# cc-ai/MUNIT

Measured on AMD Instinct MI355X. Metric: images/sec (gen_update+dis_update) @256x256 bs=8, higher is better.
Workload: dtype f32; 1 GPU; config_256.yaml AdaINGen_double+MsImageDis dis_update+gen_update, 256x256, per-GPU batch 8, fp32; global_batch=8, parallelism=dp1, gen_state=1

## Files before the change

munit_amd/csrc/conv_igemm.hip:

```cpp
#include "common.h"
#include "wino.h"
#include <cstdlib>

namespace {

struct IgemmParams {
  const float* x;
  const float* w;
  const float* bias;
  void* y;
  int B, H, W, Cin;
  int Hu, Wu, ups;
  int Ho, Wo, Cout;
  int KH, KW, stride, pad, reflect;
  int Ktot;
  long long w_row;
  long long y_sb;
  long long y_sh;
  int y_sw;
  int M;
  int act;
  float slope;
  int ps;
  long long w_phase;
// ... 952 lines not shown

int check_desc(const munit_conv_desc* d) {
  MUNIT_CHECK_ARG(d != nullptr, "conv: null descriptor");
  MUNIT_CHECK_ARG(d->B > 0 && d->H > 0 && d->W > 0 && d->Cin > 0 && d->Cout > 0, "conv: bad dims");
  MUNIT_CHECK_ARG(d->KH > 0 && d->KW > 0 && d->stride > 0 && d->pad >= 0, "conv: bad kernel geometry");
  MUNIT_CHECK_ARG(d->upsample == 0 || d->upsample == 1, "conv: upsample must be 0 or 1");
  MUNIT_CHECK_ARG(d->compute >= MUNIT_COMPUTE_F32 && d->compute <= MUNIT_COMPUTE_F32X3, "conv: bad compute mode %d", d->compute);
  MUNIT_CHECK_ARG(d->pad_mode == MUNIT_PAD_ZERO || d->pad_mode == MUNIT_PAD_REFLECT, "conv: bad pad mode");
  MUNIT_CHECK_ARG((d->in_dtype == MUNIT_DTYPE_F32 || d->in_dtype == MUNIT_DTYPE_BF16) &&
                  (d->out_dtype == MUNIT_DTYPE_F32 || d->out_dtype == MUNIT_DTYPE_BF16), "conv: bad tensor dtype");
  MUNIT_CHECK_ARG(d->in_dtype == MUNIT_DTYPE_F32 || d->Cin % 64 == 0, "conv: a bf16 input needs Cin %% 64 == 0 (got %d)", d->Cin);
  MUNIT_CHECK_ARG(d->out_dtype == MUNIT_DTYPE_F32 || d->Cout % 64 == 0, "conv: a bf16 output needs Cout %% 64 == 0 (got %d)", d->Cout);
  const int Hu = d->H << d->upsample, Wu = d->W << d->upsample;
  if (d->pad_mode == MUNIT_PAD_REFLECT)
    MUNIT_CHECK_ARG(d->pad < Hu && d->pad < Wu, "conv: reflect pad %d needs input > pad (got %dx%d)", d->pad, Hu, Wu);
  MUNIT_CHECK_ARG(Hu + 2 * d->pad >= d->KH && Wu + 2 * d->pad >= d->KW, "conv: kernel larger than padded input");
  MUNIT_CHECK_ARG((long long)d->B * Hu * Wu < (1ll << 31) / 4, "conv: too many pixels for 32-bit tile indices");
  MUNIT_CHECK_ARG((long long)d->B * (Hu + 2 * d->pad) * (Wu + 2 * d->pad) * std::max(d->Cin, d->Cout) < (1ll << 31),
                  "conv: tensor too large for the 32-bit element offsets of the tile loader");
  return MUNIT_OK;
}

}

extern "C" int munit_conv2d_out_hw(const munit_conv_desc* d, int* Ho, int* Wo) {
  int rc = check_desc(d);
  if (rc) return rc;
  *Ho = ((d->H << d->upsample) + 2 * d->pad - d->KH) / d->stride + 1;
  *Wo = ((d->W << d->upsample) + 2 * d->pad - d->KW) / d->stride + 1;
  return MUNIT_OK;
}

namespace {
bool subpixel_ok(const munit_conv_desc* d) {
  return d->upsample == 1 && d->KH == 5 && d->KW == 5 && d->pad == 2 && d->stride == 1 &&
         d->pad_mode == MUNIT_PAD_REFLECT && d->Cin % 32 == 0 && d->H >= 3 && d->W >= 3 &&
         !MUNIT_ENV_FLAG("MUNIT_DEBUG_NO_SUBPIXEL");
}
}

namespace {
__global__ void pad3to4_image_kernel(const float* __restrict__ x, f32x4* __restrict__ x4, long long npix) {
  for (long long i = (long long)blockIdx.x * blockDim.x + threadIdx.x; i < npix; i += (long long)gridDim.x * blockDim.x)
    x4[i] = f32x4{x[3 * i], x[3 * i + 1], x[3 * i + 2], 0.f};
}
__global__ void pad3to4_weight_kernel(const float* __restrict__ w, float* __restrict__ w4, int N, int taps, int kpad) {
  const long long total = (long long)N * kpad;
  for (long long i = (long long)blockIdx.x * blockDim.x + threadIdx.x; i < total; i += (long long)gridDim.x * blockDim.x) {
    const int n = (int)(i / kpad), k = (int)(i - (long long)n * kpad);
    const int tap = k >> 2, c = k & 3;
    w4[i] = (tap < taps && c < 3) ? w[((long long)n * taps + tap) * 3 + c] : 0.f;
  }
}
struct Cin4Plan {
  int kpad;
  size_t x4_bytes, w4_bytes;
};
Cin4Plan plan_cin4(long long npix, int N, int taps) {
  Cin4Plan c;
  c.kpad = (taps * 4 + BK - 1) / BK * BK;
  c.x4_bytes = align_up((size_t)npix * 4 * sizeof(float), 256);
  c.w4_bytes = align_up((size_t)N * c.kpad * sizeof(float), 256);
  return c;
}
int build_cin4(const Cin4Plan& c, const float* x3, long long npix, const float* w3, int N, int taps, void* ws, hipStream_t st) {
  f32x4* x4 = reinterpret_cast<f32x4*>(ws);
  float* w4 = reinterpret_cast<float*>(reinterpret_cast<char*>(ws) + c.x4_bytes);
  hipLaunchKernelGGL(pad3to4_image_kernel, dim3((unsigned)std::min<long long>((npix + 255) / 256, 8192)), dim3(256), 0, st, x3, x4, npix);
  MUNIT_CHECK_LAUNCH("pad3to4_image");
  hipLaunchKernelGGL(pad3to4_weight_kernel, dim3((unsigned)cdiv((long long)N * c.kpad, 256)), dim3(256), 0, st, w3, w4, N, taps, c.kpad);
  MUNIT_CHECK_LAUNCH("pad3to4_weight");
  return MUNIT_OK;
}
bool cin4_fwd_ok(const munit_conv_desc* d) {
  return d->Cin == 3 && d->in_dtype == MUNIT_DTYPE_F32 && d->upsample == 0 && d->KH * d->KW <= 64 && d->Cout % 4 == 0 &&
         NWAVES == 8 && !MUNIT_ENV_FLAG("MUNIT_DEBUG_NO_CIN4");
}

bool wino_geometry_ok(const munit_conv_desc* d) {
  return d->compute == MUNIT_COMPUTE_F32 && d->in_dtype == MUNIT_DTYPE_F32 && d->out_dtype == MUNIT_DTYPE_F32 &&
         d->KH == 3 && d->KW == 3 && d->stride == 1 && d->pad == 1 && d->upsample == 0 && d->act != MUNIT_ACT_TANH;
}
bool wino_fwd_ok(const munit_conv_desc* d) { return wino_geometry_ok(d) && munit_wino_ok(d->B, d->H, d->W, d->Cin, d->Cout); }
long long wino_s2_min_blocks() {
  static const long long v = getenv("MUNIT_WINO_S2_MIN_BLOCKS") ? atoll(getenv("MUNIT_WINO_S2_MIN_BLOCKS")) : 192;
  return v;
}
long long wino_s2_dgrad_min_blocks() {
  static const long long v = getenv("MUNIT_WINO_S2_MIN_BLOCKS") ? atoll(getenv("MUNIT_WINO_S2_MIN_BLOCKS")) : 100;
  return v;
}
bool wino_s2_fwd_ok(const munit_conv_desc* d) {
  return d->compute == MUNIT_COMPUTE_F32 && d->in_dtype == MUNIT_DTYPE_F32 && d->out_dtype == MUNIT_DTYPE_F32 && d->KH == 4 &&
         d->KW == 4 && d->stride == 2 && d->pad == 1 && d->upsample == 0 && d->act != MUNIT_ACT_TANH && d->H >= 4 && d->W >= 4 &&
         munit_wino_ok(d->B, d->H, d->W, d->Cin, d->Cout) && !MUNIT_ENV_FLAG("MUNIT_DEBUG_NO_WINOGRAD_S2") &&
         (long long)cdiv((long long)d->B * cdiv(d->H / 2, 3) * cdiv(d->W / 2, 3), 64) * (d->Cout / 64) >= wino_s2_min_blocks();
}
bool wino_s2_dgrad_ok(const munit_conv_desc* d) {
  if (!(d->compute == MUNIT_COMPUTE_F32 && d->in_dtype == MUNIT_DTYPE_F32 && d->out_dtype == MUNIT_DTYPE_F32 && d->KH == 4 &&
        d->KW == 4 && d->stride == 2 && d->pad == 1 && d->upsample == 0 && d->H >= 4 && d->W >= 4 && d->H % 2 == 0 && d->W % 2 == 0 &&
        d->Cout % 8 == 0 && d->Cin % 64 == 0 && !MUNIT_ENV_FLAG("MUNIT_DEBUG_NO_WINOGRAD_S2") && !MUNIT_ENV_FLAG("MUNIT_DEBUG_NO_WINOGRAD")))
    return false;
  const int Hd = d->H / 2, Wd = d->W / 2;
  if (d->pad_mode == MUNIT_PAD_REFLECT && (Hd % 3 == 0 || Wd % 3 == 0)) return false;
  if ((long long)d->B * d->H * d->W * std::max(d->Cin, d->Cout) >= (1ll << 29)) return false;
  return (long long)cdiv((long long)d->B * cdiv(Hd + 1, 3) * cdiv(Wd + 1, 3), 64) * (d->Cin / 64) * 4 >= wino_s2_dgrad_min_blocks();
}
bool subpixel_wino_ok(const munit_conv_desc* d) {
  return subpixel_ok(d) && d->compute == MUNIT_COMPUTE_F32 && d->in_dtype == MUNIT_DTYPE_F32 && d->out_dtype == MUNIT_DTYPE_F32 &&
         d->act != MUNIT_ACT_TANH && munit_wino_ok(d->B, d->H, d->W, d->Cin, d->Cout);
}

munit_prep_item fwd_prep_item(const munit_conv_desc* d, const float* w, float* wp) {
  munit_prep_item it{w, wp, d->Cout, d->KH, d->KW, d->Cin, MUNIT_PREP_NONE, 1, 0};
  const bool small = munit_small_fwd_supported(d) && !MUNIT_ENV_FLAG("MUNIT_DEBUG_NO_SMALL_FWD");
  if (small) return it;
  it.bf16 = d->in_dtype == MUNIT_DTYPE_BF16;
  if (subpixel_ok(d)) it.kind = subpixel_wino_ok(d) ? MUNIT_PREP_SUBPIXEL_WINOGRAD : MUNIT_PREP_SUBPIXEL;
  else if (wino_fwd_ok(d)) it.kind = MUNIT_PREP_WINOGRAD;
  else if (wino_s2_fwd_ok(d)) it.kind = MUNIT_PREP_WINOGRAD_S2;
  else if (it.bf16) it.kind = MUNIT_PREP_CAST;
  return it;
}
size_t prep_bytes(const munit_prep_item& it) {
  return it.kind == MUNIT_PREP_NONE ? 0 : align_up((size_t)prep_elems(it) * (it.bf16 ? 2 : 4), 256);
}
}

extern "C" size_t munit_conv2d_fwd_workspace_bytes(const munit_conv_desc* d) {
  int Ho, Wo;
  if (munit_conv2d_out_hw(d, &Ho, &Wo)) return 0;
  const size_t img = prep_bytes(fwd_prep_item(d, nullptr, nullptr));
  if (munit_small_fwd_supported(d) && !MUNIT_ENV_FLAG("MUNIT_DEBUG_NO_SMALL_FWD")) return munit_small_fwd_workspace(d);
  if (munit_small_fwd_supported(d) || d->in_dtype == MUNIT_DTYPE_BF16 || wino_fwd_ok(d) || wino_s2_fwd_ok(d)) return img;
  if (cin4_fwd_ok(d)) {
    const Cin4Plan c = plan_cin4((long long)d->B * d->H * d->W, d->Cout, d->KH * d->KW);
    return c.x4_bytes + c.w4_bytes;
  }
  if (subpixel_ok(d))
    return img + std::max(splitk_bytes(d->B * (4 * Wo + 4 * (Ho - 4)), d->Cout, d->KH * d->KW * d->Cin, 1),
                          splitk_bytes(d->B * (2 * Wo + 2 * (Ho - 2)), d->Cout, d->KH * d->KW * d->Cin, 1));
  return img + splitk_bytes(d->B * Ho * Wo, d->Cout, d->KH * d->KW * d->Cin, 1);
}

extern "C" int munit_conv2d_fwd(const munit_conv_desc* d, const void* x, const float* w,
                                const float* bias, void* y, void* ws, size_t ws_bytes,
                                munit_stream_t stream) {
  return munit_conv2d_fwd_prepared(d, x, w, nullptr, bias, y, ws, ws_bytes, stream);
}

extern "C" int munit_conv2d_fwd_prepared(const munit_conv_desc* d, const void* x, const float* w, const void* wp,
                                         const float* bias, void* y, void* ws, size_t ws_bytes,
                                         munit_stream_t stream) {
  int Ho, Wo;
  int rc = munit_conv2d_out_hw(d, &Ho, &Wo);
  if (rc) return rc;
  MUNIT_CHECK_ARG(x && w && y, "conv2d_fwd: null pointer");
  hipStream_t st = (hipStream_t)stream;
  if (munit_small_fwd_supported(d) && !MUNIT_ENV_FLAG("MUNIT_DEBUG_NO_SMALL_FWD")) {
    MUNIT_CHECK_ARG(d->out_dtype == MUNIT_DTYPE_F32, "conv2d_fwd: the 3-channel image head writes fp32");
    const size_t sneed = munit_small_fwd_workspace(d);
    if (sneed != 0 && (ws == nullptr || ws_bytes < sneed)) {
      munit_set_error("conv2d_fwd: workspace %zu < %zu", ws_bytes, sneed);
      return MUNIT_ERR_WORKSPACE;
    }
    return munit_small_fwd(d, Ho, Wo, x, w, bias, reinterpret_cast<float*>(y), ws, st);
  }
  const size_t need = munit_conv2d_fwd_workspace_bytes(d);
  if (need != 0 && (ws == nullptr || ws_bytes < need)) {
    munit_set_error("conv2d_fwd: workspace %zu < %zu", ws_bytes, need);
    return MUNIT_ERR_WORKSPACE;
  }
  munit_prep_item it = fwd_prep_item(d, w, reinterpret_cast<float*>(ws));
  const size_t img_bytes = prep_bytes(it);
  const float* wimg = w;
  if (it.kind != MUNIT_PREP_NONE) {
    wimg = reinterpret_cast<const float*>(wp);
    if (wimg == nullptr) {
      rc = launch_prep_one(it, st);
      if (rc) return rc;
      wimg = it.wp;
    }
  }
  if (it.kind == MUNIT_PREP_WINOGRAD_S2) {
    WinoParams q{};
    q.x = reinterpret_cast<const float*>(x); q.u = wimg; q.bias = bias; q.y = reinterpret_cast<float*>(y);
    q.y_sw = d->Cout; q.y_sh = (long long)Wo * d->Cout; q.y_sb = (long long)Ho * Wo * d->Cout;
    q.B = d->B; q.H = d->H; q.W = d->W; q.K = 4 * d->Cin; q.N = d->Cout; q.xc = d->Cin; q.cpp = d->Cin / 8;
    q.s2 = 1; q.Ho = Ho; q.Wo = Wo;
    q.x_bytes = (unsigned)((size_t)d->B * d->H * d->W * d->Cin * 4);
    q.mode = d->pad_mode == MUNIT_PAD_REFLECT ? 0 : 1;
    q.th = cdiv(Ho, 3); q.tw = cdiv(Wo, 3); q.bth = cdiv(q.th, 8); q.btw = cdiv(q.tw, 8); q.NB = d->Cout / 64;
    q.act = d->act; q.slope = d->slope;
    return munit_wino_launch(q, st);
  }
  if (it.kind == MUNIT_PREP_WINOGRAD) {
    WinoParams q{};
    q.x = reinterpret_cast<const float*>(x); q.u = wimg; q.bias = bias; q.y = reinterpret_cast<float*>(y);
    q.y_sw = d->Cout; q.y_sh = (long long)d->W * d->Cout; q.y_sb = (long long)d->H * d->W * d->Cout;
    q.B = d->B; q.H = d->H; q.W = d->W; q.K = d->Cin; q.N = d->Cout; q.xc = d->Cin; q.cpp = d->Cin / 8;
    q.x_bytes = (unsigned)((size_t)d->B * d->H * d->W * d->Cin * 4);
    q.mode = d->pad_mode == MUNIT_PAD_REFLECT ? 0 : 1;
    q.th = d->H / 2; q.tw = d->W / 2; q.bth = cdiv(q.th, 8); q.btw = cdiv(q.tw, 8); q.NB = d->Cout / 64;
    q.act = d->act; q.slope = d->slope;
    return munit_wino_launch(q, st);
  }
  void* slabs = ws ? reinterpret_cast<char*>(ws) + img_bytes : nullptr;
  const size_t slab_bytes = ws ? ws_bytes - img_bytes : 0;
  IgemmParams p{};
  p.x = reinterpret_cast<const float*>(x); p.w = wimg; p.bias = bias; p.y = y;
  p.B = d->B; p.H = d->H; p.W = d->W; p.Cin = d->Cin;
  p.ups = d->upsample; p.Hu = d->H << p.ups; p.Wu = d->W << p.ups;
  p.Ho = Ho; p.Wo = Wo; p.Cout = d->Cout;
  p.KH = d->KH; p.KW = d->KW; p.stride = d->stride; p.pad = d->pad;
  p.reflect = d->pad_mode == MUNIT_PAD_REFLECT;
  p.Ktot = d->KH * d->KW * d->Cin;
  p.w_row = p.Ktot;
  p.y_sw = d->Cout;
  p.y_sh = (long long)Wo * d->Cout;
  p.y_sb = (long long)Ho * Wo * d->Cout;
  p.M = d->B * Ho * Wo;
  p.act = d->act; p.slope = d->slope;
  p.ct = d->compute;
  p.ps = 1;
  p.bf16s = d->in_dtype == MUNIT_DTYPE_BF16;
  p.out_bf16 = d->out_dtype == MUNIT_DTYPE_BF16;
  if (cin4_fwd_ok(d)) {
    const long long npix = (long long)d->B * d->H * d->W;
    const Cin4Plan c = plan_cin4(npix, d->Cout, d->KH * d->KW);
    rc = build_cin4(c, reinterpret_cast<const float*>(x), npix, w, d->Cout, d->KH * d->KW, ws, st);
    if (rc) return rc;
    p.x = reinterpret_cast<const float*>(ws);
    p.w = reinterpret_cast<const float*>(reinterpret_cast<const char*>(ws) + c.x4_bytes);
    p.Ktot = c.kpad; p.w_row = c.kpad; p.cin4 = 1;
    return launch_igemm<0>(p, 1, st);
  }
  if (it.kind == MUNIT_PREP_SUBPIXEL || it.kind == MUNIT_PREP_SUBPIXEL_WINOGRAD) {
    IgemmParams q = p;
    int ring = 2;
    q.ups = 0; q.Hu = d->H; q.Wu = d->W;
    q.Ho = d->H; q.Wo = d->W;
    q.KH = 3; q.KW = 3; q.pad = 1; q.reflect = 0;
    q.Ktot = 9 * d->Cin; q.w_row = q.Ktot;
    q.y_sw = 2 * d->Cout;
    q.y_sh = (long long)2 * Wo * d->Cout;
    q.M = d->B * d->H * d->W;
    q.ps = 2;
    q.w_phase = (long long)d->Cout * q.Ktot;
    q.y_phase_row = (long long)Wo * d->Cout;
    q.y_phase_col = d->Cout;
    if (it.kind == MUNIT_PREP_SUBPIXEL_WINOGRAD) {
      WinoParams wq{};
      wq.x = reinterpret_cast<const float*>(x); wq.u = wimg; wq.bias = bias; wq.y = reinterpret_cast<float*>(y);
      wq.y_sw = q.y_sw; wq.y_sh = q.y_sh; wq.y_sb = p.y_sb;
      wq.u_phase = wino_image_elems(d->Cin, d->Cout); wq.y_prow = q.y_phase_row; wq.y_pcol = q.y_phase_col; wq.phases = 4;
      wq.B = d->B; wq.H = d->H; wq.W = d->W; wq.K = d->Cin; wq.N = d->Cout; wq.xc = d->Cin; wq.cpp = d->Cin / 8;
      wq.x_bytes = (unsigned)((size_t)d->B * d->H * d->W * d->Cin * 4);
      wq.mode = 1;
      wq.edge = 1;
      ring = 1;
      wq.th = d->H / 2; wq.tw = d->W / 2; wq.bth = cdiv(wq.th, 8); wq.btw = cdiv(wq.tw, 8); wq.NB = d->Cout / 64;
      wq.act = d->act; wq.slope = d->slope;
      rc = munit_wino_launch(wq, st);
    } else {
      rc = launch_igemm<0>(q, 4, st);
    }
    if (rc) return rc;
    p.frame = ring;
    p.M = d->B * (2 * ring * Wo + 2 * ring * (Ho - 2 * ring));
    p.w = it.bf16 ? reinterpret_cast<const float*>(reinterpret_cast<const bf16_t*>(wimg) + (size_t)4 * 9 * d->Cout * d->Cin) : w;
    return launch_igemm<0>(p, 1, st, slabs, slab_bytes);
  }
  return launch_igemm<0>(p, 1, st, slabs, slab_bytes);
}

namespace {
__global__ void box2x2_kernel(const f32x4* __restrict__ dy, f32x4* __restrict__ s, int B, int H, int W, int C4) {
// ... 506 lines not shown
```

munit_amd/csrc/conv_wino.hip:

```cpp
#include "wino.h"
#include <algorithm>
#include <type_traits>

namespace {

constexpr int WT = 64;
constexpr int WNB = 64;
constexpr int WK = 8;
constexpr int VBUF = 16 * WT * WK;
constexpr int UBUF = 16 * WNB * WK;
constexpr int MLD = 36;
constexpr int WINO_SMEM = 16 * WT * MLD;
static_assert(WINO_SMEM >= 2 * VBUF, "operand buffers must fit");

typedef float f32x2 __attribute__((ext_vector_type(2)));

#ifdef WINO_STAMP
__device__ long long g_wino_stamps[8 * 8 * 4];
#define WSTAMP(i) do { const long long t_ = __builtin_amdgcn_s_memtime(); st_acc[i] += t_ - st_last; st_last = t_; } while (0)
#else
#define WSTAMP(i) do { } while (0)
#endif

__device__ inline float wino_act(float v, int act, float slope) {
  return act == MUNIT_ACT_NONE ? v : (v > 0.f ? v : (act == MUNIT_ACT_RELU ? 0.f : v * slope));
}

template <int MODE, int KIND = 0>
__global__ __launch_bounds__(512) void conv_wino_kernel(WinoParams p) {
  constexpr bool REFLECT = MODE == 0;
  constexpr bool S2 = KIND == 1, DG2 = KIND == 2, UPD = KIND == 3, LIN = KIND == 1 || KIND == 2, PHK = KIND == 1 || KIND == 3;
  __shared__ __attribute__((aligned(16))) float smem[WINO_SMEM];
  const int tid = threadIdx.x, lane = tid & 63;
  const int wave = __builtin_amdgcn_readfirstlane(tid >> 6);

  int blk = blockIdx.x;
  {
    const int nb = gridDim.x, q = nb >> 3, r = nb & 7, xcd = blk & 7, idx = blk >> 3;
    blk = (xcd < r ? xcd * (q + 1) : r * (q + 1) + (xcd - r) * q) + idx;
  }
  const int n_blk = blk % p.NB;
  int m_blk = blk / p.NB;
  const int m_blk0 = m_blk;
  const int btx = m_blk % p.btw; m_blk /= p.btw;
  const int bty = m_blk % p.bth;
  const int b = m_blk / p.bth;

#ifdef WINO_SWAP_ROLES
  const bool loader = wave >= 4;
#else
  const bool loader = wave < 4;
#endif
#if defined(WINO_PRIO) && WINO_PRIO == 1
  if (!loader) __builtin_amdgcn_s_setprio(1);
#elif defined(WINO_PRIO) && WINO_PRIO == 2
  if (loader) __builtin_amdgcn_s_setprio(1);
#endif
  const int tl = (tid & 255) >> 2, cp = tid & 3;
  int gy, gx, gb = b;
  if constexpr (LIN) {
    const int t = min(m_blk0 * 64 + tl, p.B * p.th * p.tw - 1);
    gx = t % p.tw; gy = (t / p.tw) % p.th; gb = t / (p.tw * p.th);
  } else {
    gy = min(bty * 8 + (tl >> 3), p.th - 1); gx = min(btx * 8 + (tl & 7), p.tw - 1);
  }
  unsigned off[16];
  auto make_off = [&](int phase) {
    int ro[4], co[4];
#pragma unroll
    for (int i = 0; i < 4; ++i) {
      int ih, iw;
      if constexpr (S2) {
        ih = 2 * (3 * gy + i) + (phase >> 1) - 1;
        iw = 2 * (3 * gx + i) + (phase & 1) - 1;
        if (REFLECT) {
          ih = ih == -1 ? 1 : (ih == p.H ? p.H - 2 : ih);
          iw = iw == -1 ? 1 : (iw == p.W ? p.W - 2 : iw);
        }
      } else if constexpr (DG2) {
        ih = 3 * gy - 1 + i; iw = 3 * gx - 1 + i;
      } else if constexpr (UPD) {
        ih = 2 * (2 * gy + 1 + i) + (phase >> 1); iw = 2 * (2 * gx + 1 + i) + (phase & 1);
      } else {
        ih = 2 * gy - 1 + i; iw = 2 * gx - 1 + i;
        if (REFLECT) {
          ih = ih < 0 ? -ih : (ih >= p.H ? 2 * p.H - 2 - ih : ih);
          iw = iw < 0 ? -iw : (iw >= p.W ? 2 * p.W - 2 - iw : iw);
        } else if (MODE == 1 && p.edge) {
          ih = min(max(ih, 0), p.H - 1); iw = min(max(iw, 0), p.W - 1);
        }
      }
      ro[i] = (unsigned)ih < (unsigned)p.H ? (gb * p.H + ih) * p.W * p.xc : -1;
      co[i] = (unsigned)iw < (unsigned)p.W ? iw * p.xc + 2 * cp : -1;
    }
#pragma unroll
    for (int i = 0; i < 4; ++i)
#pragma unroll
      for (int j = 0; j < 4; ++j) off[i * 4 + j] = (ro[i] >= 0 && co[j] >= 0) ? (unsigned)(ro[i] + co[j]) * 4u : 0x80000000u;
  };
  unsigned* const otab = reinterpret_cast<unsigned*>(smem + 2 * VBUF) + (tid & 255);
  auto term_table = [&]() {
#pragma unroll
    for (int par = 0; par < 2; ++par)
#pragma unroll
      for (int i = 0; i < 4; ++i) {
        int ih, iw;
        if constexpr (S2) {
          ih = 2 * (3 * gy + i) + par - 1;
          iw = 2 * (3 * gx + i) + par - 1;
          if (REFLECT) {
            ih = ih == -1 ? 1 : (ih == p.H ? p.H - 2 : ih);
            iw = iw == -1 ? 1 : (iw == p.W ? p.W - 2 : iw);
          }
        } else {
          ih = 2 * (2 * gy + 1 + i) + par; iw = 2 * (2 * gx + 1 + i) + par;
        }
        otab[(par * 4 + i) * 256] = (unsigned)ih < (unsigned)p.H ? (unsigned)((gb * p.H + ih) * p.W * p.xc) * 4u : 0x80000000u;
        otab[(8 + par * 4 + i) * 256] = (unsigned)iw < (unsigned)p.W ? (unsigned)(iw * p.xc + 2 * cp) * 4u : 0x80000000u;
      }
  };
  auto load_off = [&](int phase) {
    unsigned ro[4], co[4];
#pragma unroll
    for (int i = 0; i < 4; ++i) {
      ro[i] = otab[((phase >> 1) * 4 + i) * 256];
      co[i] = otab[(8 + (phase & 1) * 4 + i) * 256];
    }
#pragma unroll
    for (int i = 0; i < 4; ++i)
#pragma unroll
      for (int j = 0; j < 4; ++j) off[i * 4 + j] = ((ro[i] | co[j]) & 0x80000000u) ? 0x80000000u : ro[i] + co[j];
  };
  if constexpr (PHK) {
    if (loader) { term_table(); load_off(0); }
  } else {
    make_off(0);
  }
  int off_phase = 0;
  const __amdgpu_buffer_rsrc_t xres = __builtin_amdgcn_make_buffer_rsrc(const_cast<float*>(p.x), 0, p.x_bytes, 0x00020000);
  f32x2 d[16];
  auto load_raw = [&](int c) {
    int cc = c;
    if constexpr (PHK) {
      const int phase = c / p.cpp;
      cc = c - phase * p.cpp;
      if (phase != off_phase) { load_off(phase); off_phase = phase; }
    }
#pragma unroll
    for (int q = 0; q < 16; ++q) d[q] = __builtin_bit_cast(f32x2, __builtin_amdgcn_raw_buffer_load_b64(xres, off[q], cc * (WK * 4), 0));
  };
  const int vpos = tl * 8 + ((cp ^ (((tl >> 3) & 1) << 1) ^ ((tl >> 4) & 3)) << 1);
  const bool e_top = gy == 0, e_bot = gy == p.th - 1, e_left = gx == 0, e_right = gx == p.tw - 1;
  auto transform_store = [&](int buf) {
    const f32x2 z = {0.f, 0.f};
    if constexpr (MODE == 2) {
#pragma unroll
      for (int j = 0; j < 4; ++j) {
        d[12 + j] += e_top ? d[4 + j] : z;
        d[0 + j] += e_bot ? d[8 + j] : z;
      }
#pragma unroll
      for (int i = 0; i < 4; ++i) {
        d[i * 4 + 3] += e_left ? d[i * 4 + 1] : z;
        d[i * 4 + 0] += e_right ? d[i * 4 + 2] : z;
      }
    }
    f32x2 u[16];
#pragma unroll
    for (int j = 0; j < 4; ++j) {
      u[0 + j] = d[0 + j] - d[8 + j];
      u[4 + j] = d[4 + j] + d[8 + j];
      u[8 + j] = d[8 + j] - d[4 + j];
      u[12 + j] = d[4 + j] - d[12 + j];
    }
    float* V = smem + buf * VBUF + vpos;
#pragma unroll
    for (int i = 0; i < 4; ++i) {
      *reinterpret_cast<f32x2*>(V + (i * 4 + 0) * 512) = u[i * 4 + 0] - u[i * 4 + 2];
      *reinterpret_cast<f32x2*>(V + (i * 4 + 1) * 512) = u[i * 4 + 1] + u[i * 4 + 2];
      *reinterpret_cast<f32x2*>(V + (i * 4 + 2) * 512) = u[i * 4 + 2] - u[i * 4 + 1];
      *reinterpret_cast<f32x2*>(V + (i * 4 + 3) * 512) = u[i * 4 + 1] - u[i * 4 + 3];
    }
  };
  const int phase = blockIdx.y;
  const f32x4* const ug = reinterpret_cast<const f32x4*>(p.u + phase * p.u_phase + (long long)n_blk * UBUF) + wave * 2 * 128 + lane;
  const long long u_chunk = (long long)p.NB * UBUF / 4;
  struct UFrag { f32x4 v[2][2]; };
  auto load_u = [&](int c, UFrag& u) {
    const f32x4* g = ug + c * u_chunk;
#pragma unroll
    for (int fq = 0; fq < 2; ++fq)
#pragma unroll
      for (int h = 0; h < 2; ++h) u.v[fq][h] = g[fq * 128 + h * 64];
  };

  f32x4 acc[2][4][4];
#pragma unroll
  for (int fq = 0; fq < 2; ++fq)
#pragma unroll
    for (int mt = 0; mt < 4; ++mt)
#pragma unroll
      for (int nt = 0; nt < 4; ++nt) acc[fq][mt][nt] = f32x4{0.f, 0.f, 0.f, 0.f};
  constexpr bool HOIST = MODE != 2;
  int fpos[2][4];
#pragma unroll
  for (int fq = 0; fq < 2; ++fq)
#pragma unroll
    for (int mt = 0; mt < 4; ++mt) {
      fpos[fq][mt] = (HOIST ? (wave * 2 + fq) * 512 : 0) + mt * 128 + (lane & 15) * 8 + (((lane >> 4) ^ (((lane >> 3) & 1) << 1) ^ mt) << 1);
      if constexpr (HOIST) asm("" : "+v"(fpos[fq][mt]));
    }
  auto compute = [&](int buf, const UFrag& u) {
    const float* Vf = smem + buf * VBUF;
    f32x2 a[2][4];
#pragma unroll
    for (int fq = 0; fq < 2; ++fq)
#pragma unroll
      for (int mt = 0; mt < 4; ++mt) {
        if constexpr (HOIST) {
          a[fq][mt] = *reinterpret_cast<const f32x2*>(Vf + fpos[fq][mt]);
        } else {
          int o = (wave * 2 + fq) * 512 + fpos[0][mt];
          asm("" : "+v"(o));
          a[fq][mt] = *reinterpret_cast<const f32x2*>(Vf + o);
        }
      }
#pragma unroll
    for (int fq = 0; fq < 2; ++fq)
#pragma unroll
      for (int t = 0; t < 2; ++t)
#pragma unroll
        for (int mt = 0; mt < 4; ++mt)
#pragma unroll
          for (int nt = 0; nt < 4; ++nt)
            acc[fq][mt][nt] = __builtin_amdgcn_mfma_f32_16x16x4f32(a[fq][mt][t], u.v[fq][nt >> 1][(nt & 1) * 2 + t], acc[fq][mt][nt], 0, 0, 0);
  };

  const int nc = p.K / WK;
#ifdef WINO_STAMP
  long long st_acc[4] = {0, 0, 0, 0};
  long long st_last = __builtin_amdgcn_s_memtime();
#endif
  if (loader) {
    UFrag u0, u1;
    load_raw(0);
    load_u(0, u0);
    transform_store(0);
    if (nc > 1) load_raw(1);
    __syncthreads();
    WSTAMP(3);
    auto body = [&](int c, int cur, const UFrag& u, UFrag& un) {
      if (c + 1 < nc) {
        load_u(c + 1, un);
        transform_store(cur ^ 1);
        if (c + 2 < nc) load_raw(c + 2);
      }
      WSTAMP(0);
      compute(cur, u);
      WSTAMP(1);
      __syncthreads();
      WSTAMP(2);
    };
    for (int c = 0; c < nc; c += 2) {
      body(c, 0, u0, u1);
      if (c + 1 < nc) body(c + 1, 1, u1, u0);
    }
  } else {
    UFrag u0, u1;
    load_u(0, u0);
    __syncthreads();
    WSTAMP(3);
    for (int c = 0; c < nc; c += 2) {
      if (c + 1 < nc) load_u(c + 1, u1);
      WSTAMP(0);
      compute(0, u0);
      WSTAMP(1);
      __syncthreads();
      WSTAMP(2);
      if (c + 1 < nc) {
        if (c + 2 < nc) load_u(c + 2, u0);
        WSTAMP(0);
        compute(1, u1);
        WSTAMP(1);
        __syncthreads();
        WSTAMP(2);
      }
    }
  }
#ifdef WINO_STAMP
  if (blockIdx.x < 8 && blockIdx.y == 0 && lane == 0)
    for (int i = 0; i < 4; ++i) g_wino_stamps[(blockIdx.x * 8 + wave) * 4 + i] = st_acc[i];
#endif
  int tid_e = tid;
  asm volatile("" : "+v"(tid_e));
  const int lane_e = tid_e & 63;
  int tw_e = p.tw, th_e = p.th;
  asm volatile("" : "+s"(tw_e), "+s"(th_e));
  const int co = tid_e & 31;
  const float slope = p.slope;
#pragma unroll
  for (int half = 0; half < 2; ++half) {
#pragma unroll
    for (int fq = 0; fq < 2; ++fq)
#pragma unroll
      for (int mt = 0; mt < 4; ++mt)
#pragma unroll
        for (int ntl = 0; ntl < 2; ++ntl)
#pragma unroll
          for (int r = 0; r < 4; ++r)
            smem[((wave * 2 + fq) * 64 + mt * 16 + 4 * (lane_e >> 4) + r) * MLD + ntl * 16 + (lane_e & 15)] = acc[fq][mt][half * 2 + ntl][r];
    __syncthreads();
    const int n = n_blk * 64 + half * 32 + co;
    const float bv = p.bias != nullptr ? p.bias[n] : 0.f;
#pragma unroll
    for (int it = 0; it < 4; ++it) {
      const int t2 = (tid_e >> 5) + 16 * it;
      float m[16];
#pragma unroll
      for (int f = 0; f < 16; ++f) m[f] = smem[(f * 64 + t2) * MLD + co];
      if constexpr (DG2) {
        float s[12];
#pragma unroll
        for (int j = 0; j < 4; ++j) {
          s[j] = (m[0 + j] + m[4 + j]) + m[8 + j];
          s[4 + j] = m[4 + j] - m[8 + j];
          s[8 + j] = (m[4 + j] + m[8 + j]) - m[12 + j];
        }
        const int t = m_blk0 * 64 + t2;
        if (t < p.B * th_e * tw_e) {
          const int tx = t % tw_e, ty = (t / tw_e) % th_e, tb = t / (tw_e * th_e);
          const int ph = phase >> 1, pw = phase & 1;
          float v[3][3];
#pragma unroll
          for (int i = 0; i < 3; ++i) {
            v[i][0] = (s[i * 4 + 0] + s[i * 4 + 1]) + s[i * 4 + 2];
            v[i][1] = s[i * 4 + 1] - s[i * 4 + 2];
            v[i][2] = (s[i * 4 + 1] + s[i * 4 + 2]) - s[i * 4 + 3];
          }
          const int fr = ph == 0 ? 0 : p.H, fc = pw == 0 ? 0 : p.W;
          if (REFLECT) {
            const int ir = fr - 3 * ty, jc = fc - 3 * tx;
#pragma unroll
            for (int j = 0; j < 3; ++j) {
              if (ph == 0) { if (ir == 0) v[1][j] += v[0][j]; }
              else { if (ir == 1) v[0][j] += v[1][j]; else if (ir == 2) v[1][j] += v[2][j]; }
            }
#pragma unroll
            for (int i = 0; i < 3; ++i) {
              if (pw == 0) { if (jc == 0) v[i][1] += v[i][0]; }
              else { if (jc == 1) v[i][0] += v[i][1]; else if (jc == 2) v[i][1] += v[i][2]; }
            }
          }
          float* yb = p.y + tb * p.y_sb + n;
#pragma unroll
          for (int i = 0; i < 3; ++i) {
            const int u = 3 * ty + i, ir = 2 * u + ph - 1;
            if (u == fr || ir < 0 || ir >= p.Ho) continue;
#pragma unroll
            for (int j = 0; j < 3; ++j) {
              const int w = 3 * tx + j, ic = 2 * w + pw - 1;
              if (w == fc || ic < 0 || ic >= p.Wo) continue;
              yb[(long long)ir * p.y_sh + (long long)ic * p.y_sw] = v[i][j];
            }
          }
        }
      } else if constexpr (S2) {
        float s[12];
#pragma unroll
        for (int j = 0; j < 4; ++j) {
          s[j] = (m[0 + j] + m[4 + j]) + m[8 + j];
          s[4 + j] = m[4 + j] - m[8 + j];
          s[8 + j] = (m[4 + j] + m[8 + j]) - m[12 + j];
        }
        const int t = m_blk0 * 64 + t2;
        if (t < p.B * th_e * tw_e) {
          const int tx = t % tw_e, ty = (t / tw_e) % th_e, tb = t / (tw_e * th_e);
          float* yp = p.y + tb * p.y_sb + (long long)(3 * ty) * p.y_sh + (long long)(3 * tx) * p.y_sw + n;
#pragma unroll
          for (int i = 0; i < 3; ++i) {
            const float v[3] = {(s[i * 4 + 0] + s[i * 4 + 1]) + s[i * 4 + 2], s[i * 4 + 1] - s[i * 4 + 2],
                                (s[i * 4 + 1] + s[i * 4 + 2]) - s[i * 4 + 3]};
#pragma unroll
            for (int j = 0; j < 3; ++j)
              if (3 * ty + i < p.Ho && 3 * tx + j < p.Wo) yp[i * p.y_sh + j * p.y_sw] = wino_act(v[j] + bv, p.act, slope);
          }
        }
      } else {
        const int ty = bty * 8 + (t2 >> 3), tx = btx * 8 + (t2 & 7);
        float s[8];
#pragma unroll
        for (int j = 0; j < 4; ++j) {
          s[j] = (m[0 + j] + m[4 + j]) + m[8 + j];
          s[4 + j] = (m[4 + j] - m[8 + j]) - m[12 + j];
        }
        if (ty < p.th && tx < p.tw) {
          const long long yo = (phase >> 1) * p.y_prow + (phase & 1) * p.y_pcol + b * p.y_sb + (long long)(2 * ty) * p.y_sh +
                               (long long)(2 * tx) * p.y_sw + n;
          float* yp = p.y + yo;
          float v0 = ((s[0] + s[1]) + s[2]) + bv, v1 = ((s[1] - s[2]) - s[3]) + bv;
          float v2 = ((s[4] + s[5]) + s[6]) + bv, v3 = ((s[5] - s[6]) - s[7]) + bv;
          if (p.add != nullptr) {
            const float* ap = p.add + yo;
            v0 += ap[0]; v1 += ap[p.y_sw]; v2 += ap[p.y_sh]; v3 += ap[p.y_sh + p.y_sw];
          }
          yp[0] = wino_act(v0, p.act, slope);
          yp[p.y_sw] = wino_act(v1, p.act, slope);
          yp[p.y_sh] = wino_act(v2, p.act, slope);
          yp[p.y_sh + p.y_sw] = wino_act(v3, p.act, slope);
        }
      }
    }
    if (half == 0) __syncthreads();
  }
}


constexpr int WG_PLANE = 4 * 64 * 2;
constexpr int WG_BUF = 16 * WG_PLANE;

template <bool S2, bool FAST, bool RING = false>
__global__ __launch_bounds__(512) void conv_wino_wgrad_kernel(WinoWgradParams p) {
  __shared__ __attribute__((aligned(16))) float smem[4 * WG_BUF];
  const int tid = threadIdx.x, lane = tid & 63;
  const int wave = __builtin_amdgcn_readfirstlane(tid >> 6);
  int blk = blockIdx.x;
  {
    const int nb = gridDim.x, q = nb >> 3, r = nb & 7, xcd = blk & 7, idx = blk >> 3;
    blk = (xcd < r ? xcd * (q + 1) : r * (q + 1) + (xcd - r) * q) + idx;
  }
  const int cib = blk % p.CB; blk /= p.CB;
  const int cob = blk % p.NB;
  const int split = blk / p.NB;
  const int phase = blockIdx.y;
  const int c_begin = split * p.cps;
  const int total_chunks = (p.tiles + 7) >> 3;
  const int nc = min(p.cps, total_chunks - c_begin);

  const __amdgpu_buffer_rsrc_t xres = __builtin_amdgcn_make_buffer_rsrc(const_cast<float*>(p.x), 0, p.x_bytes, 0x00020000);
  const __amdgpu_buffer_rsrc_t yres = __builtin_amdgcn_make_buffer_rsrc(const_cast<float*>(p.dy), 0, p.dy_bytes, 0x00020000);
  const unsigned xlane = (unsigned)(cib * 64 + lane) * 4u, ylane = (unsigned)(cob * 64 + lane) * 4u;
  const bool xside = wave < 4;
  const int pair = wave & 3;
  const bool want_db_blk = p.db_part != nullptr && cib == 0 && (!S2 || phase == 0);
  const bool want_db = want_db_blk && !xside;

  constexpr int NG = S2 ? 9 : 4;
  f32x2 d[16], g[NG];
  float dbs = 0.f;
  int cur_t = c_begin * 8 + 2 * pair, cur_tx, cur_ty, cur_b;
  {
    const int r = cur_t / p.tw;
    cur_tx = cur_t - r * p.tw; cur_b = r / p.th; cur_ty = r - cur_b * p.th;
  }
  auto load_raw = [&](int c) {
    (void)c;
#pragma unroll
    for (int e = 0; e < 2; ++e) {
      const int t = cur_t + e;
      if (FAST || (S2 && RING) || t < p.tiles) {
        int tx = cur_tx + e, ty = cur_ty, b = cur_b;
// ... 282 lines not shown
      *o = beta == 0.f ? v[s] : beta * *o + v[s];
    }
  }
}

}

#ifdef WINO_STAMP
extern "C" int munit_debug_wino_stamps(long long* host_out) {
  return hipMemcpyFromSymbol(host_out, HIP_SYMBOL(g_wino_stamps), sizeof(long long) * 8 * 8 * 4) == hipSuccess ? 0 : -1;
}
#endif

bool munit_wino_wgrad_ok(int B, int H, int W, int Cin, int Cout) {
  if (MUNIT_ENV_FLAG("MUNIT_DEBUG_NO_WINOGRAD") || MUNIT_ENV_FLAG("MUNIT_DEBUG_NO_WINOGRAD_WGRAD")) return false;
  return Cin % 64 == 0 && Cout % 64 == 0 && H % 2 == 0 && W % 2 == 0 && H >= 2 && W >= 2 &&
         (long long)B * H * W * std::max(Cin, Cout) < (1ll << 29);
}

int munit_wino_wgrad_splits(long long tiles, int Cin, int Cout, int phases) {
  const int chunks = cdiv(tiles, 8);
  const int pairs = (Cin / 64) * (Cout / 64) * std::max(1, phases);
  int ksplit = std::max(1, std::min(chunks, cdiv(256, pairs)));
  const int cps = cdiv(chunks, ksplit);
  return cdiv(chunks, cps);
}

size_t munit_wino_wgrad_workspace(long long tiles, int Cin, int Cout, int phases) {
  const size_t k = (size_t)munit_wino_wgrad_splits(tiles, Cin, Cout, phases) * std::max(1, phases);
  return align_up(k * 16 * Cin * Cout * sizeof(float), 256) + align_up(k * Cout * sizeof(float), 256);
}

int munit_wino_wgrad_launch(WinoWgradParams p, float* dw, long long dw_phase, float* db, float beta, float beta_b, void* ws,
                            hipStream_t st) {
  p.phases = std::max(1, p.phases);
  p.tiles = p.B * p.th * p.tw;
  p.ksplit = munit_wino_wgrad_splits(p.tiles, p.Cin, p.Cout, p.phases);
  p.cps = cdiv(cdiv(p.tiles, 8), p.ksplit);
  p.CB = p.Cin / 64; p.NB = p.Cout / 64;
  p.slab = reinterpret_cast<float*>(ws);
  float* db_part = reinterpret_cast<float*>(reinterpret_cast<char*>(ws) +
                                            align_up((size_t)p.ksplit * p.phases * 16 * p.Cin * p.Cout * sizeof(float), 256));
  p.db_part = db != nullptr ? db_part : nullptr;
  const dim3 grid((unsigned)(p.CB * p.NB * p.ksplit), (unsigned)p.phases);
  bool fast = p.tiles % 8 == 0 && !MUNIT_ENV_FLAG("MUNIT_DEBUG_NO_WINO_WGRAD_FAST");
  if (p.s2) fast = fast && p.reflect && p.H % 6 == 0 && p.W % 6 == 0 && p.Ho % 3 == 0 && p.Wo % 3 == 0;
  else fast = fast && (p.xo == -1 ? (p.reflect && p.H >= 2 && p.W >= 2 && 2 * p.th <= p.H && 2 * p.tw <= p.W)
                                  : (p.xo >= 0 && 2 * (p.th - 1) + p.xo + 3 < p.H && 2 * (p.tw - 1) + p.xo + 3 < p.W));
  if (p.s2) {
    const bool xclamp = !fast && p.reflect == 1 && p.tiles % 8 == 0 && p.H >= 2 && p.W >= 2 && !MUNIT_ENV_FLAG("MUNIT_DEBUG_NO_WINO_WGRAD_FAST");
    if (fast) hipLaunchKernelGGL((conv_wino_wgrad_kernel<true, true>), grid, dim3(512), 0, st, p);
    else if (xclamp) hipLaunchKernelGGL((conv_wino_wgrad_kernel<true, false, true>), grid, dim3(512), 0, st, p);
    else hipLaunchKernelGGL((conv_wino_wgrad_kernel<true, false>), grid, dim3(512), 0, st, p);
  } else if (p.ring_mask) {
    MUNIT_CHECK_ARG(p.reflect == 2 && p.xo == -1 && p.phases == 4, "conv_wino_wgrad: ring_mask goes with the replicated edge and 4 phases");
    if (fast) hipLaunchKernelGGL((conv_wino_wgrad_kernel<false, true, true>), grid, dim3(512), 0, st, p);
    else hipLaunchKernelGGL((conv_wino_wgrad_kernel<false, false, true>), grid, dim3(512), 0, st, p);
  } else {
    MUNIT_CHECK_ARG(p.reflect != 2, "conv_wino_wgrad: the replicated edge goes with ring_mask");
    if (fast) hipLaunchKernelGGL((conv_wino_wgrad_kernel<false, true>), grid, dim3(512), 0, st, p);
    else hipLaunchKernelGGL((conv_wino_wgrad_kernel<false, false>), grid, dim3(512), 0, st, p);
  }
  MUNIT_CHECK_LAUNCH("conv_wino_wgrad");
  const int pair_blocks = cdiv((long long)p.Cout * p.Cin, 256);
  const int bias_blocks = db != nullptr ? cdiv(p.Cout, 256) : 0;
  hipLaunchKernelGGL(wino_wgrad_reduce_kernel, dim3((unsigned)(pair_blocks + bias_blocks), (unsigned)p.phases), dim3(256), 0, st, p.slab,
                     db_part, dw, dw_phase, db, p.Cout, p.Cin, p.ksplit, beta, beta_b, pair_blocks, p.s2);
  MUNIT_CHECK_LAUNCH("wino_wgrad_reduce");
  return MUNIT_OK;
}

bool munit_wino_ok(int B, int H, int W, int K, int N) {
  if (MUNIT_ENV_FLAG("MUNIT_DEBUG_NO_WINOGRAD")) return false;
  return K % 8 == 0 && N % 64 == 0 && H % 2 == 0 && W % 2 == 0 && H >= 2 && W >= 2 &&
         (long long)B * H * W * K < (1ll << 29) && (long long)B * H * W * N < (1ll << 40);
}

int munit_wino_launch(const WinoParams& p, hipStream_t st) {
  const bool lin = p.s2 == 1 || p.s2 == 2;
  const long long blocks = lin ? (long long)cdiv((long long)p.B * p.th * p.tw, 64) * p.NB : (long long)p.B * p.bth * p.btw * p.NB;
  MUNIT_CHECK_ARG(blocks > 0 && blocks < (1ll << 31), "conv_wino: bad grid");
  const dim3 grid((unsigned)blocks, (unsigned)std::max(1, p.phases));
  if (p.s2 == 1) {
    if (p.mode == 0) hipLaunchKernelGGL((conv_wino_kernel<0, 1>), grid, dim3(512), 0, st, p);
    else hipLaunchKernelGGL((conv_wino_kernel<1, 1>), grid, dim3(512), 0, st, p);
    MUNIT_CHECK_LAUNCH("conv_wino_s2");
    return MUNIT_OK;
  }
  if (p.s2 == 3) {
    hipLaunchKernelGGL((conv_wino_kernel<1, 3>), grid, dim3(512), 0, st, p);
    MUNIT_CHECK_LAUNCH("conv_wino_up_dgrad");
    return MUNIT_OK;
  }
  if (p.s2 == 2) {
    if (p.mode == 0) hipLaunchKernelGGL((conv_wino_kernel<0, 2>), grid, dim3(512), 0, st, p);
    else hipLaunchKernelGGL((conv_wino_kernel<1, 2>), grid, dim3(512), 0, st, p);
    MUNIT_CHECK_LAUNCH("conv_wino_s2_dgrad");
    return MUNIT_OK;
  }
  if (p.mode == 0) hipLaunchKernelGGL(conv_wino_kernel<0>, grid, dim3(512), 0, st, p);
  else if (p.mode == 1) hipLaunchKernelGGL(conv_wino_kernel<1>, grid, dim3(512), 0, st, p);
  else hipLaunchKernelGGL(conv_wino_kernel<2>, grid, dim3(512), 0, st, p);
  MUNIT_CHECK_LAUNCH("conv_wino");
  return MUNIT_OK;
}
```

munit_amd/csrc/wino.h:

```cpp
#pragma once
#include "common.h"

__host__ __device__ inline long long wino_image_elems(int K, int N) { return 16ll * K * N; }

__device__ inline float wino_u_of_g(const float (&g)[3][3], int f) {
  const int fi = f >> 2, fj = f & 3;
  float t[3];
#pragma unroll
  for (int s = 0; s < 3; ++s) {
    const float a = g[0][s], b = g[1][s], cc = g[2][s];
    t[s] = fi == 0 ? a : fi == 1 ? 0.5f * ((a + cc) + b) : fi == 2 ? 0.5f * ((a + cc) - b) : cc;
  }
  return fj == 0 ? t[0] : fj == 1 ? 0.5f * ((t[0] + t[2]) + t[1]) : fj == 2 ? 0.5f * ((t[0] + t[2]) - t[1]) : t[2];
}

__device__ inline void wino_item_index(long long j, int N, int& k, int& no) {
  const int NB = N >> 6;
  const int w = (int)(j & 511);
  const int e = w & 1, ntl = (w >> 1) & 1, l = (w >> 2) & 63, h = w >> 8;
  const long long rest = j >> 9;
  const int nb = (int)(rest % NB), c = (int)(rest / NB);
  k = c * 8 + 2 * (l >> 4) + e;
  no = nb * 64 + (2 * h + ntl) * 16 + (l & 15);
}
// ... 55 lines not shown
    for (int b = 0; b < 2; ++b) g[a][b] = w[(((long long)k * 4 + 2 * (1 - a) + ph) * 4 + 2 * (1 - b) + pw) * Cin + no];
  float t[4][2];
#pragma unroll
  for (int b = 0; b < 2; ++b) {
    t[0][b] = g[0][b];
    t[1][b] = 0.5f * (g[0][b] + g[1][b]);
    t[2][b] = 0.5f * (g[0][b] - g[1][b]);
    t[3][b] = g[1][b];
  }
  float* o = img + phase * wino_image_elems(Cout, Cin) + (jj >> 9) * (16 * 512) + (jj & 511);
#pragma unroll
  for (int fi = 0; fi < 4; ++fi) {
    o[(fi * 4 + 0) * 512] = t[fi][0];
    o[(fi * 4 + 1) * 512] = 0.5f * (t[fi][0] + t[fi][1]);
    o[(fi * 4 + 2) * 512] = 0.5f * (t[fi][0] - t[fi][1]);
    o[(fi * 4 + 3) * 512] = t[fi][1];
  }
}

__device__ inline void wino_subpixel_dgrad_weight_item(const float* __restrict__ w, float* __restrict__ img, int Cout, int Cin, long long j) {
  int k, no;
  wino_item_index(j, Cin, k, no);
  const int ph = k / Cout, co = k - ph * Cout, a = ph >> 1, b = ph & 1;
  float g[3][3];
#pragma unroll
  for (int r = 0; r < 3; ++r)
#pragma unroll
    for (int sft = 0; sft < 3; ++sft) {
      const int dh = 2 - r, dw = 2 - sft;
      const int h0 = a == 0 ? (dh == 0 ? 0 : dh == 1 ? 2 : 4) : (dh == 0 ? 0 : dh == 1 ? 1 : 3);
      const int hn = a == 0 ? (dh == 2 ? 1 : 2) : (dh == 0 ? 1 : 2);
      const int w0 = b == 0 ? (dw == 0 ? 0 : dw == 1 ? 2 : 4) : (dw == 0 ? 0 : dw == 1 ? 1 : 3);
      const int wn = b == 0 ? (dw == 2 ? 1 : 2) : (dw == 0 ? 1 : 2);
      float sum = 0.f;
      for (int kh = h0; kh < h0 + hn; ++kh)
        for (int kw = w0; kw < w0 + wn; ++kw) sum += w[(((long long)co * 5 + kh) * 5 + kw) * Cin + no];
      g[r][sft] = sum;
    }
  wino_store_item(img, j, g);
}

__device__ inline void wino_subpixel_weight_item(const float* __restrict__ w, float* __restrict__ img, int Cout, int Cin, long long j) {
  const long long per = (long long)Cin * Cout;
  const int ph = (int)(j / per), a = ph >> 1, b = ph & 1;
  int k, no;
  wino_item_index(j - ph * per, Cout, k, no);
  float g[3][3];
#pragma unroll
  for (int dh = 0; dh < 3; ++dh)
#pragma unroll
    for (int dw = 0; dw < 3; ++dw) {
      const int h0 = a == 0 ? (dh == 0 ? 0 : dh == 1 ? 2 : 4) : (dh == 0 ? 0 : dh == 1 ? 1 : 3);
      const int hn = a == 0 ? (dh == 2 ? 1 : 2) : (dh == 0 ? 1 : 2);
      const int w0 = b == 0 ? (dw == 0 ? 0 : dw == 1 ? 2 : 4) : (dw == 0 ? 0 : dw == 1 ? 1 : 3);
      const int wn = b == 0 ? (dw == 2 ? 1 : 2) : (dw == 0 ? 1 : 2);
      float s = 0.f;
      for (int kh = h0; kh < h0 + hn; ++kh)
        for (int kw = w0; kw < w0 + wn; ++kw) s += w[(((long long)no * 5 + kh) * 5 + kw) * Cin + k];
      g[dh][dw] = s;
    }
  wino_store_item(img + ph * wino_image_elems(Cin, Cout), j - ph * per, g);
}

struct WinoParams {
  const float* x;
  const float* u;
  const float* bias;
  const float* add;
  float* y;
  long long y_sb, y_sh, y_sw;
  long long u_phase, y_prow, y_pcol;
  int phases;
  unsigned x_bytes;
  int B, H, W, K, N;
  int xc, cpp;
  int s2, Ho, Wo;
  int mode;
  int edge;
  int th, tw;
  int bth, btw;
  int NB;
  int act;
  float slope;
};

bool munit_wino_ok(int B, int H, int W, int K, int N);
int munit_wino_launch(const WinoParams& p, hipStream_t st);

struct WinoWgradParams {
  const float* x;
  const float* dy;
  float* slab;
  float* db_part;
  unsigned x_bytes, dy_bytes;
  long long dy_sb, dy_sh, dy_sw, dy_off;
  long long dy_prow, dy_pcol;
  int B, H, W, Cin, Cout;
  int reflect;
  int ring_mask;
  int xo;
  int th, tw, tiles;
  int cps;
  int CB, NB, ksplit;
  int phases;
  int s2, Ho, Wo;
};
bool munit_wino_wgrad_ok(int B, int H, int W, int Cin, int Cout);
int munit_wino_wgrad_splits(long long tiles, int Cin, int Cout, int phases);
size_t munit_wino_wgrad_workspace(long long tiles, int Cin, int Cout, int phases);
int munit_wino_wgrad_launch(WinoWgradParams p, float* dw, long long dw_phase, float* db, float beta, float beta_b, void* ws,
                            hipStream_t st);
```

Baseline: 78.95 images/s.

## Add split-K to stride-2 Winograd forward conv and lower its block threshold

Adds a split-K path to the stride-2 4x4 Winograd forward kernel: when few output blocks exist, the contraction over input channel chunks is split across blockIdx.z. Each split writes partial sums to a workspace slab, and an existing split-K epilogue kernel then reduces them and applies bias and activation. The minimum block threshold for taking the Winograd path drops from 192 to 36, so smaller downsampling convs now use it too. The trade is more parallelism on small layers against extra slab memory traffic and one more kernel launch.

```diff
diff --git a/munit_amd/csrc/conv_igemm.hip b/munit_amd/csrc/conv_igemm.hip
--- a/munit_amd/csrc/conv_igemm.hip
+++ b/munit_amd/csrc/conv_igemm.hip
@@ -1058,19 +1058,45 @@
          d->KH == 3 && d->KW == 3 && d->stride == 1 && d->pad == 1 && d->upsample == 0 && d->act != MUNIT_ACT_TANH;
 }
 bool wino_fwd_ok(const munit_conv_desc* d) { return wino_geometry_ok(d) && munit_wino_ok(d->B, d->H, d->W, d->Cin, d->Cout); }
+constexpr long long WINO_S2_FWD_FULL_BLOCKS = 192;
+constexpr long long WINO_S2_FWD_MIN_BLOCKS = 36;
+constexpr int WINO_S2_FWD_MIN_CHUNKS = 8;
 long long wino_s2_min_blocks() {
-  static const long long v = getenv("MUNIT_WINO_S2_MIN_BLOCKS") ? atoll(getenv("MUNIT_WINO_S2_MIN_BLOCKS")) : 192;
+  static const long long v = getenv("MUNIT_WINO_S2_MIN_BLOCKS") ? atoll(getenv("MUNIT_WINO_S2_MIN_BLOCKS")) : WINO_S2_FWD_MIN_BLOCKS;
+  return v;
+}
+int wino_s2_min_chunks() {
+  static const int v = getenv("MUNIT_WINO_S2_MIN_CHUNKS") ? std::max(1, atoi(getenv("MUNIT_WINO_S2_MIN_CHUNKS"))) : WINO_S2_FWD_MIN_CHUNKS;
   return v;
 }
 long long wino_s2_dgrad_min_blocks() {
   static const long long v = getenv("MUNIT_WINO_S2_MIN_BLOCKS") ? atoll(getenv("MUNIT_WINO_S2_MIN_BLOCKS")) : 100;
   return v;
+}
+long long wino_s2_fwd_blocks(const munit_conv_desc* d) {
+  return (long long)cdiv((long long)d->B * cdiv(d->H / 2, 3) * cdiv(d->W / 2, 3), 64) * (d->Cout / 64);
+}
+struct WinoS2Split { int ks, cps; };
+WinoS2Split wino_s2_fwd_split(const munit_conv_desc* d) {
+  const long long blocks = wino_s2_fwd_blocks(d);
+  const int nc = d->Cin / 2;
+  WinoS2Split s{1, nc};
+  if (blocks >= WINO_S2_FWD_FULL_BLOCKS || MUNIT_ENV_FLAG("MUNIT_DEBUG_NO_SPLITK")) return s;
+  const int ks = (int)std::min<long long>(256 / blocks, nc / wino_s2_min_chunks());
+  if (ks <= 1) return s;
+  s.cps = cdiv(nc, ks);
+  s.ks = cdiv(nc, s.cps);
+  return s;
+}
+size_t wino_s2_fwd_slab_bytes(const munit_conv_desc* d) {
+  const WinoS2Split s = wino_s2_fwd_split(d);
+  return s.ks > 1 ? align_up((size_t)s.ks * d->B * (d->H / 2) * (d->W / 2) * d->Cout * sizeof(float), 256) : 0;
 }
 bool wino_s2_fwd_ok(const munit_conv_desc* d) {
   return d->compute == MUNIT_COMPUTE_F32 && d->in_dtype == MUNIT_DTYPE_F32 && d->out_dtype == MUNIT_DTYPE_F32 && d->KH == 4 &&
          d->KW == 4 && d->stride == 2 && d->pad == 1 && d->upsample == 0 && d->act != MUNIT_ACT_TANH && d->H >= 4 && d->W >= 4 &&
          munit_wino_ok(d->B, d->H, d->W, d->Cin, d->Cout) && !MUNIT_ENV_FLAG("MUNIT_DEBUG_NO_WINOGRAD_S2") &&
-         (long long)cdiv((long long)d->B * cdiv(d->H / 2, 3) * cdiv(d->W / 2, 3), 64) * (d->Cout / 64) >= wino_s2_min_blocks();
+         wino_s2_fwd_blocks(d) >= wino_s2_min_blocks();
 }
 bool wino_s2_dgrad_ok(const munit_conv_desc* d) {
   if (!(d->compute == MUNIT_COMPUTE_F32 && d->in_dtype == MUNIT_DTYPE_F32 && d->out_dtype == MUNIT_DTYPE_F32 && d->KH == 4 &&
@@ -1108,7 +1134,8 @@
   if (munit_conv2d_out_hw(d, &Ho, &Wo)) return 0;
   const size_t img = prep_bytes(fwd_prep_item(d, nullptr, nullptr));
   if (munit_small_fwd_supported(d) && !MUNIT_ENV_FLAG("MUNIT_DEBUG_NO_SMALL_FWD")) return munit_small_fwd_workspace(d);
-  if (munit_small_fwd_supported(d) || d->in_dtype == MUNIT_DTYPE_BF16 || wino_fwd_ok(d) || wino_s2_fwd_ok(d)) return img;
+  if (wino_s2_fwd_ok(d)) return img + wino_s2_fwd_slab_bytes(d);
+  if (munit_small_fwd_supported(d) || d->in_dtype == MUNIT_DTYPE_BF16 || wino_fwd_ok(d)) return img;
   if (cin4_fwd_ok(d)) {
     const Cin4Plan c = plan_cin4((long long)d->B * d->H * d->W, d->Cout, d->KH * d->KW);
     return c.x4_bytes + c.w4_bytes;
@@ -1168,7 +1195,21 @@
     q.mode = d->pad_mode == MUNIT_PAD_REFLECT ? 0 : 1;
     q.th = cdiv(Ho, 3); q.tw = cdiv(Wo, 3); q.bth = cdiv(q.th, 8); q.btw = cdiv(q.tw, 8); q.NB = d->Cout / 64;
     q.act = d->act; q.slope = d->slope;
-    return munit_wino_launch(q, st);
+    const WinoS2Split sp = wino_s2_fwd_split(d);
+    if (sp.ks <= 1) return munit_wino_launch(q, st);
+    float* slab = reinterpret_cast<float*>(reinterpret_cast<char*>(ws) + img_bytes);
+    q.y = slab; q.bias = nullptr; q.act = MUNIT_ACT_NONE;
+    q.ksplit = sp.ks; q.cps = sp.cps; q.y_split = (long long)d->B * Ho * Wo * d->Cout;
+    rc = munit_wino_launch(q, st);
+    if (rc) return rc;
+    IgemmParams e{};
+    e.slab = slab; e.ksplit = sp.ks; e.M = d->B * Ho * Wo; e.Cout = d->Cout; e.Ho = Ho; e.Wo = Wo; e.ps = 1;
+    e.bias = bias; e.y = y; e.act = d->act; e.slope = d->slope;
+    e.y_sw = d->Cout; e.y_sh = (long long)Wo * d->Cout; e.y_sb = (long long)Ho * Wo * d->Cout;
+    const long long total = (long long)e.M * e.Cout;
+    hipLaunchKernelGGL(splitk_epilogue_kernel, dim3((unsigned)std::min<long long>((total + 255) / 256, 4096)), dim3(256), 0, st, e, 1);
+    MUNIT_CHECK_LAUNCH("splitk_epilogue");
+    return MUNIT_OK;
   }
   if (it.kind == MUNIT_PREP_WINOGRAD) {
     WinoParams q{};
diff --git a/munit_amd/csrc/conv_wino.hip b/munit_amd/csrc/conv_wino.hip
--- a/munit_amd/csrc/conv_wino.hip
+++ b/munit_amd/csrc/conv_wino.hip
@@ -45,6 +45,13 @@
   const int btx = m_blk % p.btw; m_blk /= p.btw;
   const int bty = m_blk % p.bth;
   const int b = m_blk / p.bth;
+  int c0 = 0, c1 = p.K / WK;
+  int ph0 = 0;
+  if constexpr (KIND == 1) {
+    c0 = __builtin_amdgcn_readfirstlane(blockIdx.z * p.cps);
+    c1 = __builtin_amdgcn_readfirstlane(min(c0 + p.cps, c1));
+    ph0 = (c0 >= p.cpp) + (c0 >= 2 * p.cpp) + (c0 >= 3 * p.cpp);
+  }
 
 #ifdef WINO_SWAP_ROLES
   const bool loader = wave >= 4;
@@ -132,11 +139,11 @@
       for (int j = 0; j < 4; ++j) off[i * 4 + j] = ((ro[i] | co[j]) & 0x80000000u) ? 0x80000000u : ro[i] + co[j];
   };
   if constexpr (PHK) {
-    if (loader) { term_table(); load_off(0); }
+    if (loader) { term_table(); load_off(ph0); }
   } else {
     make_off(0);
   }
-  int off_phase = 0;
+  int off_phase = ph0;
   const __amdgpu_buffer_rsrc_t xres = __builtin_amdgcn_make_buffer_rsrc(const_cast<float*>(p.x), 0, p.x_bytes, 0x00020000);
   f32x2 d[16];
   auto load_raw = [&](int c) {
@@ -236,24 +243,23 @@
             acc[fq][mt][nt] = __builtin_amdgcn_mfma_f32_16x16x4f32(a[fq][mt][t], u.v[fq][nt >> 1][(nt & 1) * 2 + t], acc[fq][mt][nt], 0, 0, 0);
   };
 
-  const int nc = p.K / WK;
 #ifdef WINO_STAMP
   long long st_acc[4] = {0, 0, 0, 0};
   long long st_last = __builtin_amdgcn_s_memtime();
 #endif
   if (loader) {
     UFrag u0, u1;
-    load_raw(0);
-    load_u(0, u0);
+    load_raw(c0);
+    load_u(c0, u0);
     transform_store(0);
-    if (nc > 1) load_raw(1);
+    if (c0 + 1 < c1) load_raw(c0 + 1);
     __syncthreads();
     WSTAMP(3);
     auto body = [&](int c, int cur, const UFrag& u, UFrag& un) {
-      if (c + 1 < nc) {
+      if (c + 1 < c1) {
         load_u(c + 1, un);
         transform_store(cur ^ 1);
-        if (c + 2 < nc) load_raw(c + 2);
+        if (c + 2 < c1) load_raw(c + 2);
       }
       WSTAMP(0);
       compute(cur, u);
@@ -261,24 +267,24 @@
       __syncthreads();
       WSTAMP(2);
     };
-    for (int c = 0; c < nc; c += 2) {
+    for (int c = c0; c < c1; c += 2) {
       body(c, 0, u0, u1);
-      if (c + 1 < nc) body(c + 1, 1, u1, u0);
+      if (c + 1 < c1) body(c + 1, 1, u1, u0);
     }
   } else {
     UFrag u0, u1;
-    load_u(0, u0);
+    load_u(c0, u0);
     __syncthreads();
     WSTAMP(3);
-    for (int c = 0; c < nc; c += 2) {
-      if (c + 1 < nc) load_u(c + 1, u1);
+    for (int c = c0; c < c1; c += 2) {
+      if (c + 1 < c1) load_u(c + 1, u1);
       WSTAMP(0);
       compute(0, u0);
       WSTAMP(1);
       __syncthreads();
       WSTAMP(2);
-      if (c + 1 < nc) {
-        if (c + 2 < nc) load_u(c + 2, u0);
+      if (c + 1 < c1) {
+        if (c + 2 < c1) load_u(c + 2, u0);
         WSTAMP(0);
         compute(1, u1);
         WSTAMP(1);
@@ -375,7 +381,7 @@
         const int t = m_blk0 * 64 + t2;
         if (t < p.B * th_e * tw_e) {
           const int tx = t % tw_e, ty = (t / tw_e) % th_e, tb = t / (tw_e * th_e);
-          float* yp = p.y + tb * p.y_sb + (long long)(3 * ty) * p.y_sh + (long long)(3 * tx) * p.y_sw + n;
+          float* yp = p.y + (long long)blockIdx.z * p.y_split + tb * p.y_sb + (long long)(3 * ty) * p.y_sh + (long long)(3 * tx) * p.y_sw + n;
 #pragma unroll
           for (int i = 0; i < 3; ++i) {
             const float v[3] = {(s[i * 4 + 0] + s[i * 4 + 1]) + s[i * 4 + 2], s[i * 4 + 1] - s[i * 4 + 2],
@@ -824,8 +830,14 @@
   MUNIT_CHECK_ARG(blocks > 0 && blocks < (1ll << 31), "conv_wino: bad grid");
   const dim3 grid((unsigned)blocks, (unsigned)std::max(1, p.phases));
   if (p.s2 == 1) {
-    if (p.mode == 0) hipLaunchKernelGGL((conv_wino_kernel<0, 1>), grid, dim3(512), 0, st, p);
-    else hipLaunchKernelGGL((conv_wino_kernel<1, 1>), grid, dim3(512), 0, st, p);
+    WinoParams q = p;
+    const int nc = p.K / WK;
+    if (q.ksplit <= 1) { q.ksplit = 1; q.cps = nc; q.y_split = 0; }
+    MUNIT_CHECK_ARG(q.cps > 0 && (long long)(q.ksplit - 1) * q.cps < nc && (long long)q.ksplit * q.cps >= nc && q.ksplit <= 65535,
+                    "conv_wino: bad split of the contraction (%d x %d chunks of %d)", q.ksplit, q.cps, nc);
+    const dim3 sgrid((unsigned)blocks, 1, (unsigned)q.ksplit);
+    if (p.mode == 0) hipLaunchKernelGGL((conv_wino_kernel<0, 1>), sgrid, dim3(512), 0, st, q);
+    else hipLaunchKernelGGL((conv_wino_kernel<1, 1>), sgrid, dim3(512), 0, st, q);
     MUNIT_CHECK_LAUNCH("conv_wino_s2");
     return MUNIT_OK;
   }
diff --git a/munit_amd/csrc/wino.h b/munit_amd/csrc/wino.h
--- a/munit_amd/csrc/wino.h
+++ b/munit_amd/csrc/wino.h
@@ -161,6 +161,8 @@
   int NB;
   int act;
   float slope;
+  int ksplit, cps;
+  long long y_split;
 };
 
 bool munit_wino_ok(int B, int H, int W, int K, int N);
```

Result: no change. 79.11 images/s (median of 6 runs) (+0.2%).
